# hzyu17/GaussianVI

Measured on AMD Instinct MI355X. Metric: sigma-point psi-evals/sec + NGD iters/sec, 1024-factor d=12 p=5 chain, higher is better.
Workload: dtype f64; 1 GPU; c3: T=1025 states, n=6; 1 step = 1 device-resident NGD iteration; restart every 30; factor_sets_columns=[K factors, d, GH degree p, N sigma points], factor_set_kinds=1024 x quadratic-prior d=12 p=5 (N=17217); 1025 x fixed-prior d=6 p=5 (N=1433), kernel_variant=6, chunks_per_factor=4, fused_pass=True, one_launch_factor_stage=False, mirror_pairs=False, fuse_trial=2

## Files before the change

gaussianvi_amd/csrc/chain_launch.hpp:

```cpp
#pragma once
#include <hip/hip_runtime.h>

#include <algorithm>
#include <atomic>
#include <vector>

#include "kernels_chain.hpp"
#include "kernels_chain_wave.hpp"

namespace gvi {

struct ChainPass { int level0, m, S, top, first, par, lp_off, blocks; };
struct ChainPlan { std::vector<ChainPass> passes; int threads = 0; };

inline int chain_padded(int n) {
  for (int N : {1, 2, 3, 4, 6, 8, 12, 16}) if (n <= N) return n >= 1 ? N : 0;
  return 0;
}
inline bool chain_supported(int n) { return chain_padded(n) != 0; }

inline int chain_levels(int T) {
  int L = 0;
  while ((1 << L) < T) ++L;
  return L;
// ... 20 lines not shown
  return p;
}

template <int N>
inline hipError_t chain_allow_lds() {
  static bool done[64] = {};
  int dev = 0;
  hipError_t e = hipGetDevice(&dev);
  if (e != hipSuccess) return e;
  if (dev >= 0 && dev < 64 && done[dev]) return hipSuccess;
  const int lim = 160 * 1024;
  if ((e = hipFuncSetAttribute((const void*)chain_forward_kernel<N, false>, hipFuncAttributeMaxDynamicSharedMemorySize, lim)) != hipSuccess) return e;
  if ((e = hipFuncSetAttribute((const void*)chain_forward_kernel<N, true>, hipFuncAttributeMaxDynamicSharedMemorySize, lim)) != hipSuccess) return e;
  if ((e = hipFuncSetAttribute((const void*)chain_backward_kernel<N>, hipFuncAttributeMaxDynamicSharedMemorySize, lim)) != hipSuccess) return e;
  if ((e = hipFuncSetAttribute((const void*)chain_top_back_kernel<N>, hipFuncAttributeMaxDynamicSharedMemorySize, lim)) != hipSuccess) return e;
  if (dev >= 0 && dev < 64) done[dev] = true;
  return hipSuccess;
}

struct ChainSync { unsigned* words = nullptr; unsigned seq = 0; unsigned fault = 0; };

template <int N>
inline hipError_t chain_launch_t(const ChainPlan& pl, ChainArgs a0, ChainArgs a1, bool on0, bool on1, hipStream_t st, const AsmList& AL,
                                 const ChainSync& sync) {
  hipError_t e = chain_allow_lds<N>();
  if (e != hipSuccess) return e;
  auto set = [](ChainArgs& a, const ChainPass& ps) {
    a.level0 = ps.level0; a.m = ps.m; a.S = ps.S; a.first = ps.first; a.par = ps.par; a.lp_off = ps.lp_off;
  };
  a0.sync = a1.sync = nullptr; a0.sync_seq = a1.sync_seq = 0; a0.sync_fault = a1.sync_fault = sync.fault;
  const bool back0 = on0 && a0.need_back;
  const int npass = (int)pl.passes.size();
  bool merged = false;
  if (sync.words && npass >= 2 && (back0 || on1)) {
    const ChainPass& pt = pl.passes[npass - 1];
    const ChainPass& pc = pl.passes[npass - 2];
    size_t lds = 0;
    if (on0) lds = std::max(lds, chain::fwd_lds_doubles<true, false, true, N>(pt.S));
    if (on1) lds = std::max(lds, chain::fwd_lds_doubles<false, true, true, N>(pt.S));
    if (back0) lds = std::max(lds, chain::bwd_lds_doubles<true, N>(pc.S));
    if (on1) lds = std::max(lds, chain::bwd_lds_doubles<false, N>(pc.S));
    merged = lds * 8 <= 160 * 1024;
  }
  for (const ChainPass& ps : pl.passes) {
    set(a0, ps); set(a1, ps);
    if (ps.top && merged) {
      const ChainPass& pc = pl.passes[npass - 2];
      size_t lds = 0;
      if (on0) lds = std::max(lds, chain::fwd_lds_doubles<true, false, true, N>(ps.S));
      if (on1) lds = std::max(lds, chain::fwd_lds_doubles<false, true, true, N>(ps.S));
      if (back0) lds = std::max(lds, chain::bwd_lds_doubles<true, N>(pc.S));
      if (on1) lds = std::max(lds, chain::bwd_lds_doubles<false, N>(pc.S));
      lds *= 8;
      a0.sync = sync.words; a1.sync = sync.words + 1; a0.sync_seq = a1.sync_seq = sync.seq;
      const int nb0 = on0 ? 1 : 0, nbt = nb0 + (on1 ? 1 : 0);
      const int nb0c = back0 ? pc.blocks : 0, nbc = nb0c + (on1 ? pc.blocks : 0);
      const ChainPassDev cp{pc.level0, pc.m, pc.S, pc.first, pc.par, pc.lp_off};
      hipLaunchKernelGGL((chain_top_back_kernel<N>), dim3(nbt + nbc), dim3(pl.threads), lds, st, a0, a1, nb0, AL, cp, nbt, nb0c);
      a0.sync = a1.sync = nullptr;
      continue;
    }
    size_t lds = 0;
    if (ps.top) {
      if (on0) lds = std::max(lds, chain::fwd_lds_doubles<true, false, true, N>(ps.S));
      if (on1) lds = std::max(lds, chain::fwd_lds_doubles<false, true, true, N>(ps.S));
    } else {
      if (on0) lds = std::max(lds, chain::fwd_lds_doubles<true, false, false, N>(ps.S));
      if (on1) lds = std::max(lds, chain::fwd_lds_doubles<false, true, false, N>(ps.S));
    }
    lds *= 8;
    if (lds > 160 * 1024) return hipErrorInvalidValue;
    const int nb0 = on0 ? ps.blocks : 0, nb = nb0 + (on1 ? ps.blocks : 0);
    if (ps.top) hipLaunchKernelGGL((chain_forward_kernel<N, true>), dim3(nb), dim3(pl.threads), lds, st, a0, a1, nb0, AL);
    else hipLaunchKernelGGL((chain_forward_kernel<N, false>), dim3(nb), dim3(pl.threads), lds, st, a0, a1, nb0, AL);
  }
  if (back0 || on1) {
    for (int i = npass - 2 - (merged ? 1 : 0); i >= 0; --i) {
      const ChainPass& ps = pl.passes[i];
      set(a0, ps); set(a1, ps);
      size_t lds = 0;
      if (back0) lds = std::max(lds, chain::bwd_lds_doubles<true, N>(ps.S));
      if (on1) lds = std::max(lds, chain::bwd_lds_doubles<false, N>(ps.S));
      lds *= 8;
      if (lds > 160 * 1024) return hipErrorInvalidValue;
      const int nb0 = back0 ? ps.blocks : 0, nb = nb0 + (on1 ? ps.blocks : 0);
      hipLaunchKernelGGL((chain_backward_kernel<N>), dim3(nb), dim3(pl.threads), lds, st, a0, a1, nb0);
    }
  }
  return hipGetLastError();
}

inline bool& chain_wave_enabled() { static bool on = true; return on; }
inline bool chain_wave_applies(int T, int n) { return chain_wave_enabled() && n >= 1 && n <= chain_wave::WN && T >= 1 && T <= chain_wave::WT_MAX; }

inline bool& chain_asm_dense_enabled() { static bool on = true; return on; }

inline std::atomic<long long>* chain_asm_launches() { static std::atomic<long long> c[2]; return c; }

inline hipError_t chain_launch(int n, const ChainPlan& pl, ChainArgs a0, ChainArgs a1, bool on0, bool on1, hipStream_t st,
                               const AsmList* AL = nullptr, const ChainSync& sync = ChainSync{}) {
  a0.n = a1.n = n;
  AsmList none{};
  const AsmList& L = AL ? *AL : none;
  if (!AL) a0.asm_on = a1.asm_on = 0;
  else if (chain_asm_dense_enabled() && chain_asm_dense(L, n) && (on0 ? a0.T : a1.T) > 1) {
    if (a0.asm_on) a0.asm_on = ASM_DENSE;
    if (a1.asm_on) a1.asm_on = ASM_DENSE;
    ++chain_asm_launches()[0];
  } else ++chain_asm_launches()[1];
  if (chain_wave_applies(on0 ? a0.T : a1.T, n)) {
    const int nb0 = on0 ? 1 : 0, nb = nb0 + (on1 ? 1 : 0);
    if (nb == 0) return hipSuccess;
    hipLaunchKernelGGL(chain_wave_kernel, dim3(nb), dim3(64), 0, st, a0, a1, nb0, L);
    return hipGetLastError();
  }
  switch (chain_padded(n)) {
// ... 14 lines not shown
```

gaussianvi_amd/csrc/gvi_hip.hip:

```cpp
#include "../../include/gvi_hip.h"

#include <hip/hip_runtime.h>
#include <hip/hip_ext.h>
#include <dlfcn.h>

#include <algorithm>
#include <chrono>
#include <cassert>
#include <cmath>
#include <cstdio>
#include <cstdlib>
#include <cstring>
#include <memory>
#include <map>
#include <set>
#include <string>
#include <thread>
#include <vector>

#include "host_linalg.hpp"
#include "kernels_bt.hpp"
#include "chain_launch.hpp"
#include "kernels_factor.hpp"
#include "kernels_orbit.hpp"
// ... 1009 lines not shown
  if (e != hipSuccess || ndev <= 0)
    return fail(nullptr, GVI_ERR_HIP, "no HIP device: this library has no CPU fallback");
  if (device < 0 || device >= ndev) return fail(nullptr, GVI_ERR_ARG, "device index out of range");
  if (hipSetDevice(device) != hipSuccess) return fail(nullptr, GVI_ERR_HIP, "hipSetDevice failed");
  std::unique_ptr<gvi_ctx> c(new gvi_ctx);
  c->device = device; c->dtype = dtype;
  if (hipStreamCreateWithFlags(&c->stream, hipStreamNonBlocking) != hipSuccess)
    return fail(nullptr, GVI_ERR_HIP, "hipStreamCreate failed");
  if (const char* w = getenv("GVI_NO_SCOST")) c->no_scost = atoi(w) != 0;
  if (const char* w = getenv("GVI_ORBIT")) c->orbit = atoi(w) != 0;
  if (const char* w = getenv("GVI_FUSED")) c->fused = atoi(w) != 0;
  if (const char* w = getenv("GVI_ASM_ON_LOAD")) c->asm_on_load = atoi(w) != 0;
  if (const char* w = getenv("GVI_PIPELINE")) c->pipeline = atoi(w) != 0;
  if (const char* w = getenv("GVI_CHAIN_WAVE")) chain_wave_enabled() = atoi(w) != 0;
  if (const char* w = getenv("GVI_ASM_DENSE")) chain_asm_dense_enabled() = atoi(w) != 0;
  if (const char* w = getenv("GVI_CHAIN_MERGE")) c->chain_merge = atoi(w) != 0;
  if (const char* w = getenv("GVI_SREG_PIPE")) c->sreg_pipe = atoi(w) != 0;
  if (const char* w = getenv("GVI_MIRROR")) c->mirror = atoi(w) != 0;
  if (const char* w = getenv("GVI_NO_PAIR")) c->pair_fuse = atoi(w) == 0;
  if (const char* w = getenv("GVI_NO_FUSE_GATHER")) c->fuse_gather = atoi(w) == 0;
  if (const char* w = getenv("GVI_SIDE_SOLVE")) c->side_solve = atoi(w) != 0;
  if (const char* w = getenv("GVI_FUSE_TRIAL")) c->fuse_trial = std::min(2, std::max(0, atoi(w)));
  if (const char* w = getenv("GVI_SPIN_MS")) c->spin_ms = std::max(0, atoi(w));
  if (const char* w = getenv("GVI_SAFE_PUBLISH")) c->safe_publish = atoi(w) != 0;
  if (hipEventCreateWithFlags(&c->fork, hipEventDisableTiming) != hipSuccess ||
      hipHostMalloc((void**)&c->host_slot, 128, hipHostMallocMapped | hipHostMallocCoherent) != hipSuccess ||
      hipHostGetDevicePointer((void**)&c->host_slot_dev, c->host_slot, 0) != hipSuccess)
    return fail(nullptr, GVI_ERR_HIP, "event / host-mapped slot allocation failed");
  for (int q = 0; q < 16; ++q) c->host_slot[q] = 0.0;
  *out = c.release();
// ... 2214 lines not shown
  else if (n == "sreg_pipe") ctx->sreg_pipe = value != 0;
  else if (n == "mirror") ctx->mirror = value != 0;
  else if (n == "pair_fuse") ctx->pair_fuse = value != 0;
  else if (n == "fuse_gather") ctx->fuse_gather = value != 0;
  else if (n == "side_solve") ctx->side_solve = value != 0;
  else if (n == "dual_chain") ctx->dual_chain = value != 0;
  else if (n == "warm_start") ctx->warm_start = value != 0;
  else if (n == "no_scost") ctx->no_scost = value != 0;
  else if (n == "target_waves") ctx->target_waves = std::max(1, value);
  else if (n == "orbit") ctx->orbit = value != 0;
  else if (n == "fused") ctx->fused = value != 0;
  else if (n == "assemble_on_load") ctx->asm_on_load = value != 0;
  else if (n == "pipeline") ctx->pipeline = value != 0;
  else if (n == "chain_wave") chain_wave_enabled() = value != 0;
  else if (n == "asm_dense") chain_asm_dense_enabled() = value != 0;
  else if (n == "sample_sweep") ctx->sample_sweep = value != 0;
  else if (n == "solve_lds") ctx->solve_lds = value != 0;
  else if (n == "chain_merge") { ctx->chain_merge = value != 0; ctx->chain_merge_fault = value == 2; }
  else if (n == "trust_table_degree") ctx->trust_table_degree = value != 0;
  else if (n == "safe_publish") {
    GVICK(sync(ctx));
    ctx->safe_publish = value != 0;
    for (int q = 0; q < 16; ++q) ctx->host_slot[q] = 0.0;
  }
  else if (n == "chol_sqrt") { ctx->chol_sqrt = value != 0; for (auto& s : ctx->sets) s->use_chol = ctx->chol_sqrt; }
  else if (n == "jacobi_tol_exp") {
    if (value > -20) return fail(ctx, GVI_ERR_ARG, "jacobi_tol_exp must be <= -20 (threshold 10^value on squared magnitudes)");
    ctx->jacobi_tol = std::pow(10.0, (double)value);
    for (auto& s : ctx->sets) s->jtol = ctx->jacobi_tol;
  }
// ... 330 lines not shown
```

gaussianvi_amd/csrc/kernels_chain.hpp:

```cpp
#pragma once
#include <hip/hip_runtime.h>
#include <stdint.h>

#include "device_common.hpp"
#include "kernels_bt.hpp"

namespace gvi {

constexpr int CHAIN_MATS = 10;
constexpr int CHAIN_VECS = 5;

__host__ __device__ inline size_t chain_lp_entries(int T) { return (size_t)2 * T + 1024; }
__host__ __device__ inline size_t chain_ws_doubles(int T, int n) {
  return (size_t)CHAIN_MATS * T * n * n + (size_t)CHAIN_VECS * T * n + chain_lp_entries(T);
}

struct ChainArgs {
  int T;
  int n;
  int level0;
  int m;
  int S;
  int first;
  int par;
  int need_back;
  int lp_off;
  const double* D;
  const double* U;
  const double* rhs;
  double rhs_scale;
  double* ws;
  int* wsi;
  double* SigD;
  double* SigU;
  double* x;
  double* hld;
  const double* mixV;
  double* mixOut;
  double mix_step;
  int asm_on;
  double* asmD;
// ... 187 lines not shown
}

__device__ __forceinline__ void st_out(double* p, const double v, const bool wt) {
  if (wt) __hip_atomic_store(p, v, __ATOMIC_RELAXED, __HIP_MEMORY_SCOPE_AGENT);
  else *p = v;
}

__device__ __forceinline__ double readlane64(double v, int src) {
  union { double d; int i[2]; } u;
  u.d = v;
  u.i[0] = __builtin_amdgcn_readlane(u.i[0], src);
  u.i[1] = __builtin_amdgcn_readlane(u.i[1], src);
  return u.d;
}

template <int N> __device__ __forceinline__ int ext_el(const int n, const int el) {
  if (n == N) return el;
  const int r = el / N, c = el % N;
  return (r < n && c < n) ? r * n + c : -1;
}

template <int N> __device__ __forceinline__ double* ws_mat(const ChainArgs& a, int idx) { return a.ws + (size_t)idx * a.T * (N * N); }
template <int N> __device__ __forceinline__ double* ws_vec(const ChainArgs& a, int idx) {
  return a.ws + (size_t)CHAIN_MATS * a.T * (N * N) + (size_t)idx * a.T * N;
}
template <int N> __device__ __forceinline__ double* ws_lp(const ChainArgs& a) { return ws_vec<N>(a, CHAIN_VECS); }
enum { W_E = 0, W_GA = 1, W_GB = 2, W_NU = 3, W_DEFF = 4, W_LS = 5 , W_RS = 7, W_SL = 8, W_SR = 9 };
enum { V_V = 0, V_YLS = 1 , V_YRS = 3, V_YEFF = 4 };

struct LogPiv {
// ... 9 lines not shown
  static constexpr int cY = cB + N;
  static constexpr int NC = cY + (HAS_Y ? 1 : 0);
  static_assert(NC <= 64, "tile does not fit one wave");
};

struct ElimIO {
  int oD, oR;
  int oUa, oUb;
  int oRa, oDb;
  int oNU;
  int oy, oyR, oyRa, oyb;
  int oZero;
  int oEl, oGAl, oGBl, ovl;
};

template <bool PIVOT, bool HAS_E, bool HAS_Y, bool TOP, int N>
__device__ __forceinline__ void eliminate(double* sm, const int lane, const ElimIO io, double* gE, double* gGA, double* gGB,
                                          double* gv, double* gNU, LogPiv& lp) {
  using C = Cols<HAS_E, HAS_Y, N>;
  const bool has_a = io.oUa >= 0, has_b = io.oUb >= 0;
  const bool isD = lane < N;
  const bool isE = HAS_E && lane >= C::cE && lane < C::cA;
  const bool isA = lane >= C::cA && lane < C::cB;
  const bool isB = lane >= C::cB && lane < C::cY;
  const bool isY = HAS_Y && lane == C::cY;
  const int cc = isD ? lane : (isE ? lane - C::cE : (isA ? lane - C::cA : (isB ? lane - C::cB : 0)));
  int p0 = io.oZero, s0 = 0, p1 = io.oZero;
  if (isD) { p0 = io.oD + cc * N; s0 = 1; p1 = io.oR + cc * N; }
  else if (isA) { if (has_a) { p0 = io.oUa + cc; s0 = N; } }
  else if (isB) { if (has_b) { p0 = io.oUb + cc * N; s0 = 1; } }
  else if (isY) { p0 = io.oy; s0 = 1; p1 = io.oyR; }
  CHAIN_STAMP(TOP && HAS_E);
  double col[N];
#pragma unroll
  for (int r = 0; r < N; ++r) col[r] = sm[p0 + r * s0] + sm[p1 + r];
  CHAIN_STAMP(TOP && HAS_E);
  if (HAS_E) {
#pragma unroll
    for (int r = 0; r < N; ++r) col[r] = isE ? (r == cc ? 1.0 : 0.0) : col[r];
  }
  constexpr int RB = chain_threads(N) == 1024 ? 128 : 256;
  constexpr bool PRE = N * N * 2 <= (RB == 128 ? 72 : 100);
  double uap[PRE ? N : 1][N];
  if (PRE && has_a) {
#pragma unroll
    for (int k = 0; k < (PRE ? N : 1); ++k) ld_row<N>(sm + io.oUa + k * N, uap[k]);
  }
  double pivs[N];
  int bad = 0;
#pragma unroll
  for (int p = 0; p < N; ++p) {
    if (PIVOT) {
      double best = fabs(col[p]);
      int rs = p;
#pragma unroll
      for (int r = p + 1; r < N; ++r) {
        const bool gt = fabs(col[r]) > best;
        best = gt ? fabs(col[r]) : best;
        rs = gt ? r : rs;
      }
      rs = fabs(col[p]) * 8.0 >= best ? p : rs;
      rs = __builtin_amdgcn_readlane(rs, p);
      if (rs != p) {
#pragma unroll
// ... 5 lines not shown
    double ap[N];
#pragma unroll
    for (int r = 0; r < N; ++r) ap[r] = readlane64(col[r], p);
    const double piv = ap[p];
    if (!(piv > 0.0)) bad = 1;
    pivs[p] = piv;
    double ip = __builtin_amdgcn_rcp(piv);
    ip = fma(fma(-piv, ip, 1.0), ip, ip);
    ip = fma(fma(-piv, ip, 1.0), ip, ip);
    const double f = col[p] * ip;
#pragma unroll
    for (int r = 0; r < N; ++r)
      if (r != p) col[r] = fma(-ap[r], f, col[r]);
    col[p] = f;
  }
  CHAIN_STAMP(TOP && HAS_E);
  {
    double mp = 1.0;
    int es = 0;
#pragma unroll
    for (int p = 0; p < N; ++p) {
      mp *= __builtin_amdgcn_frexp_mant(pivs[p]);
      es += __builtin_amdgcn_frexp_exp(pivs[p]);
    }
    const double t = lp.m * mp;
    lp.m = __builtin_amdgcn_frexp_mant(t);
    lp.e += es + __builtin_amdgcn_frexp_exp(t);
    lp.bad |= bad;
  }
  CHAIN_STAMP(TOP && HAS_E);
  if (TOP) {
    if (lane >= N && lane < C::NC) {
      const int o = isE ? io.oEl + cc : (isA ? io.oGAl + cc : (isB ? io.oGBl + cc : io.ovl));
      const int so = isY ? 1 : N;
#pragma unroll
      for (int r = 0; r < N; ++r) sm[o + r * so] = col[r];
    }
  } else {
    if (lane >= N && lane < C::NC) {
      double* g = isE ? gE + cc * N : (isA ? gGA + cc * N : (isB ? gGB + cc * N : gv));
      st_row<N>(g, col);
    }
  }
  CHAIN_STAMP(TOP && HAS_E);
  constexpr bool UBPRE = N * N * 2 <= (RB == 128 ? 32 : 100);
  double t[N], ub[UBPRE ? N : 1][N];
#pragma unroll
  for (int r = 0; r < N; ++r) t[r] = 0.0;
#pragma unroll
  for (int k = 0; k < N; ++k) {
    if (has_a) {
      double ua[N];
      if (PRE) {
#pragma unroll
// ... 34 lines not shown
#pragma unroll
        for (int k = 0; k < N; ++k) ubr[k] = ubl[UBLATE ? r : 0][k];
      } else ld_row<N>(sm + io.oUb + r * N, ubr);
      double acc = 0.0;
#pragma unroll
      for (int k = 0; k < N; ++k) acc = fma(-ubr[k], col[k], acc);
      s[r] = acc;
    }
    if (isB || isY) {
      double* o = sm + (isY ? io.oyb : io.oDb + cc * N);
#pragma unroll
      for (int r = 0; r < N; ++r) lds_add(o + r, s[r]);
    }
  }
  CHAIN_STAMP(TOP && HAS_E);
}

template <int N>
__device__ __forceinline__ void marginal_node(double* sm, const int lane, const bool has_b, const int oE, const int oGA, const int oGB,
                                              const int oSaa, const int oSbb, const int oX, const int oY, const int oSee,
                                              const int oSL, const int oSLt, const int oSR, const int oSRt, double* gSee, double* gSL,
                                              double* gSR, double* gUa, double* gUe, const int n,
                                              [[maybe_unused]] const bool stamp = false, const bool wt = false) {
  constexpr int nn = N * N, R = (nn + 63) / 64;
  double slv[R], srv[R];
  CHAIN_STAMP(stamp);
#pragma unroll
  for (int q = 0; q < R; ++q) {
    const int el = q * 64 + lane;
    const bool on = el < nn;
// ... 44 lines not shown
    if (has_b) {
      ld_row<N>(sm + oSR + r * N, u);
      ld_row<N>(sm + oGB + c * N, w);
#pragma unroll
      for (int k = 0; k < N; ++k) see = fma(-u[k], w[k], see);
    }
    if (on) {
      sm[oSee + el] = see;
      if (r < n && c < n) st_out(gSee + r * n + c, see, wt);
    }
  }
  CHAIN_STAMP(stamp);
}

template <bool HAS_E, bool HAS_Y, bool TOP, int N>
__host__ __device__ constexpr size_t fwd_lds_doubles(int S) {
  constexpr int nn = N * N;
  size_t w = (size_t)2 * (S + 1) * nn + (size_t)2 * S * nn;
  if (TOP) w += (size_t)3 * S * nn + (HAS_E ? (size_t)S * nn : 0);
  if (HAS_Y) w += (size_t)2 * (S + 1) * N + (TOP ? (size_t)(2 * S + 1) * N : 0);
  return w + N + (N & 1) + 128;
}
template <bool HAS_E, int N>
__host__ __device__ constexpr size_t bwd_lds_doubles(int S) {
  constexpr int nn = N * N;
  return (HAS_E ? (size_t)5 * (S + 1) * nn + (size_t)3 * S * nn
                : (size_t)(S + 1) * N + (size_t)S * N + (size_t)2 * S * nn)
         + 2;
}

__device__ __forceinline__ void chain_signal(unsigned* sync, const unsigned seq) {
  if (!sync) return;
  asm volatile("s_waitcnt vmcnt(0)" ::: "memory");
  __syncthreads();
  if (threadIdx.x == 0) __hip_atomic_store(sync, seq, __ATOMIC_RELAXED, __HIP_MEMORY_SCOPE_AGENT);
}
// ... 10 lines not shown
    *lds_word = ok;
  }
  __syncthreads();
  return *lds_word != 0;
}
__device__ __forceinline__ double chain_ld(const double* p, const bool fresh) {
  return fresh ? __hip_atomic_load(p, __ATOMIC_RELAXED, __HIP_MEMORY_SCOPE_AGENT) : *p;
}

__device__ __forceinline__ bool pred_fail_here(LazyPred& p) {
  __builtin_amdgcn_sched_barrier(0);
  asm volatile("" : "+v"(p.v));
  return pred_fail(p);
}

template <bool PIVOT, bool HAS_E, bool HAS_Y, bool TOP, int N>
__device__ __forceinline__ void forward_body(const ChainArgs& a, const AsmList& AL, const int bid, double* sm) {
  constexpr int nn = N * N;
  LazyPred lpred = pred_issue(a.pred, a.pred_val);
  const int T = a.T, S = a.S, st = 1 << a.level0;
  const int tid = threadIdx.x, wave = __builtin_amdgcn_readfirstlane(tid >> 6), lane = tid & 63, nwaves = blockDim.x >> 6, nthr = blockDim.x;
  const int x0 = bid * S * st;
  const int oDl = 0;
  const int oRl = oDl + (S + 1) * nn;
  const int oCt = oRl + (S + 1) * nn;
  const int oNU = oCt + S * nn;
  const int oEl = oNU + S * nn;
  const int oGAl = oEl + (TOP ? S * nn : 0);
  const int oGBl = oGAl + (TOP ? S * nn : 0);
  const int oSRt = oGBl + (TOP ? S * nn : 0);
  const int oyl = oSRt + ((TOP && HAS_E) ? S * nn : 0);
  const int oyR = oyl + (HAS_Y ? (S + 1) * N : 0);
  const int ovl = oyR + (HAS_Y ? (S + 1) * N : 0);
  const int oxl = ovl + ((HAS_Y && TOP) ? S * N : 0);
  const int oZero = oxl + ((HAS_Y && TOP) ? (S + 1) * N : 0);
  const int oRed = oZero + N + (N & 1);
  CHAIN_STAMP(TOP && HAS_E);
  const int cnt = min(S, (T - x0 + st - 1) >> a.level0);
  const int xn = x0 + S * st;
  const bool ext_right = !TOP && xn < T;
  const bool first = a.first != 0;
  const bool mix = first && (a.mixV != nullptr || (a.asm_on && !HAS_Y));
  [[maybe_unused]] double lpm = 1.0;
  [[maybe_unused]] int lpe = 0, lpb = 0;
  if constexpr (TOP) {
    if (a.hld) {
      for (int t = tid; t < a.lp_off; t += nthr) {
        const double mv = ws_lp<N>(a)[t];
        const int eb = a.wsi[t];
        const double pr = lpm * mv;
        lpm = __builtin_amdgcn_frexp_mant(pr);
// ... 169 lines not shown
#pragma unroll
      for (int o = 32; o > 0; o >>= 1) {
        const double t = lpm * __shfl_xor(lpm, o);
        lpe += __shfl_xor(lpe, o) + __builtin_amdgcn_frexp_exp(t);
        lpm = __builtin_amdgcn_frexp_mant(t);
        lpb |= __shfl_xor(lpb, o);
      }
      if (lane == 0) { sm[oRed + 64 + wave] = lpm; ((int*)(sm + oRed + 96))[wave] = lpe * 2 + lpb; }
    }
  }
  LogPiv lp;
  lp.m = 1.0; lp.e = 0; lp.bad = 0;
  for (int lam = 0; lam < a.m; ++lam) {
    const int h2 = 1 << lam;
    const int nel = (cnt + h2 - 1) >> (lam + 1);
    for (int u = wave; u < nel; u += nwaves) {
      const int j = (2 * u + 1) * h2, x = x0 + j * st;
      const int ja = j - h2, jb = j + h2;
      const bool has_b = (jb < cnt) || (jb == S && ext_right);
      ElimIO io;
      io.oD = oDl + j * nn; io.oR = oRl + j * nn;
      io.oUa = lam == 0 ? oCt + ja * nn : oNU + (j - h2 / 2) * nn;
      io.oUb = !has_b ? -1 : (lam == 0 ? oCt + j * nn : oNU + (j + h2 / 2) * nn);
      io.oRa = oRl + ja * nn; io.oDb = oDl + jb * nn;
      io.oNU = oNU + j * nn;
      io.oy = oyl + j * N; io.oyR = oyR + j * N; io.oyRa = oyR + ja * N; io.oyb = oyl + jb * N;
      io.oZero = oZero;
      io.oEl = oEl + j * nn; io.oGAl = oGAl + j * nn; io.oGBl = oGBl + j * nn; io.ovl = ovl + j * N;
      const size_t gx = (size_t)x * nn;
      double* gNU = (!TOP && lam == a.m - 1 && has_b) ? ws_mat<N>(a, W_NU) + gx : nullptr;
      eliminate<PIVOT, HAS_E, HAS_Y, TOP, N>(sm, lane, io, ws_mat<N>(a, W_E) + gx, ws_mat<N>(a, W_GA) + gx, ws_mat<N>(a, W_GB) + gx,
                                             ws_vec<N>(a, V_V) + (size_t)x * N, gNU, lp);
    }
    lds_barrier();
    CHAIN_STAMP(TOP && HAS_E);
  }
  if (!TOP) {
    for (int el = tid; el < nn; el += nthr) {
      ws_mat<N>(a, W_RS)[(size_t)x0 * nn + el] = sm[oRl + el];
      if (ext_right) ws_mat<N>(a, W_LS + a.par)[(size_t)xn * nn + el] = sm[oDl + S * nn + el];
    }
    if (HAS_Y && tid < N) {
      ws_vec<N>(a, V_YRS)[(size_t)x0 * N + tid] = sm[oyR + tid];
      if (ext_right) ws_vec<N>(a, V_YLS + a.par)[(size_t)xn * N + tid] = sm[oyl + S * N + tid];
    }
    if (lane == 0) {
      const int ent = a.lp_off + bid * nwaves + wave;
      ws_lp<N>(a)[ent] = lp.m;
      a.wsi[ent] = lp.e * 2 + lp.bad;
    }
    return;
  }
  if constexpr (TOP) {
    if (wave == 0) {
      ElimIO io;
      io.oD = oDl; io.oR = oRl; io.oUa = -1; io.oUb = -1; io.oRa = 0; io.oDb = 0; io.oNU = 0;
      io.oy = oyl; io.oyR = oyR; io.oyRa = 0; io.oyb = 0; io.oZero = oZero;
      io.oEl = oEl; io.oGAl = oGAl; io.oGBl = oGBl; io.ovl = ovl;
      eliminate<PIVOT, HAS_E, HAS_Y, true, N>(sm, lane, io, nullptr, nullptr, nullptr, nullptr, nullptr, lp);
    }
    int* redi = (int*)(sm + oRed + 32);
    if (a.hld && lane == 0) { sm[oRed + wave] = lp.m; redi[wave] = lp.e * 2 + lp.bad; }
    lds_barrier();
    if (a.hld && wave == nwaves - 1) {
      const int* redi2 = (const int*)(sm + oRed + 96);
      const int k2 = lane & 31;
      const bool on = k2 < nwaves;
      double mv = on ? (lane < 32 ? sm[oRed + k2] : sm[oRed + 64 + k2]) : 1.0;
      int eb = on ? (lane < 32 ? redi[k2] : redi2[k2]) : 0;
      int ev = eb >> 1, bflag = eb & 1;
#pragma unroll
      for (int o = 32; o > 0; o >>= 1) {
        const double t = mv * __shfl_xor(mv, o);
        ev += __shfl_xor(ev, o) + __builtin_amdgcn_frexp_exp(t);
// ... 214 lines not shown
      }
      lds_barrier();
    }
  }
}

}


template <int N, bool TOP>
__global__ __launch_bounds__(chain_threads(N)) void chain_forward_kernel(ChainArgs a0, ChainArgs a1, int nb0, AsmList AL) {
  extern __shared__ double sm[];
  constexpr int KA_LINES = (2 * sizeof(ChainArgs) + 8 + sizeof(AsmList) + 63) / 64;
  static_assert(KA_LINES == 13, "kernarg_warm: one specialisation per argument block size");
  kernarg_warm<KA_LINES>();
  if ((int)blockIdx.x < nb0) chain::forward_body<false, true, false, TOP, N>(a0, AL, (int)blockIdx.x, sm);
  else chain::forward_body<true, false, true, TOP, N>(a1, AL, (int)blockIdx.x - nb0, sm);
}

template <int N>
__global__ __launch_bounds__(chain_threads(N)) void chain_backward_kernel(ChainArgs a0, ChainArgs a1, int nb0) {
  extern __shared__ double sm[];
  constexpr int KA_LINES = (2 * sizeof(ChainArgs) + 4 + 63) / 64;
  static_assert(KA_LINES == 7, "kernarg_warm: one specialisation per argument block size");
  kernarg_warm<KA_LINES>();
  if ((int)blockIdx.x < nb0) chain::backward_body<true, false, N>(a0, (int)blockIdx.x, sm);
  else chain::backward_body<false, true, N>(a1, (int)blockIdx.x - nb0, sm);
}

template <int N>
__global__ __launch_bounds__(chain_threads(N)) void chain_top_back_kernel(ChainArgs a0, ChainArgs a1, int nb0, AsmList AL, ChainPassDev cp,
                                                                           int nbt, int nb0c) {
  extern __shared__ double sm[];
  constexpr int KA_LINES = (2 * sizeof(ChainArgs) + 8 + sizeof(AsmList) + sizeof(ChainPassDev) + 8 + 63) / 64;
  static_assert(KA_LINES == 14, "kernarg_warm: one specialisation per argument block size");
  kernarg_warm<KA_LINES>();
  const int b = (int)blockIdx.x;
  if (b < nbt) {
    if (b < nb0) chain::forward_body<false, true, false, true, N>(a0, AL, b, sm);
    else chain::forward_body<true, false, true, true, N>(a1, AL, b - nb0, sm);
    return;
  }
  const int bc = b - nbt;
  ChainArgs c = bc < nb0c ? a0 : a1;
  c.level0 = cp.level0; c.m = cp.m; c.S = cp.S; c.first = cp.first; c.par = cp.par; c.lp_off = cp.lp_off;
  if (bc < nb0c) chain::backward_body<true, false, N>(c, bc, sm);
  else chain::backward_body<false, true, N>(c, bc - nb0c, sm);
}

}
```

Before: 211.4 billion psi-evals/s.

## Add DPP row-broadcast Gauss-Jordan elimination with two eliminations per wave for n=6 chain

For padded block size 6, adds a new elimination path. Gauss-Jordan pivot broadcasts use DPP row_newbcast moves and fused v_fmac_f64_dpp instead of the previous per-pivot readlane-style broadcast. Columns are packed into a two-row 16-lane layout so each 64-lane wave handles two eliminations at once. The pivot log-determinant products are reduced through a small LDS scratch area. The old kernels are kept as readlane variants and selected per pass based on the ratio of eliminations to waves, and the feature can be toggled by env var or setting. This adds inline asm with s_nop hazard padding, extra LDS, and more template specialisations.

```diff
diff --git a/gaussianvi_amd/csrc/chain_launch.hpp b/gaussianvi_amd/csrc/chain_launch.hpp
--- a/gaussianvi_amd/csrc/chain_launch.hpp
+++ b/gaussianvi_amd/csrc/chain_launch.hpp
@@ -58,6 +58,11 @@
   if ((e = hipFuncSetAttribute((const void*)chain_forward_kernel<N, true>, hipFuncAttributeMaxDynamicSharedMemorySize, lim)) != hipSuccess) return e;
   if ((e = hipFuncSetAttribute((const void*)chain_backward_kernel<N>, hipFuncAttributeMaxDynamicSharedMemorySize, lim)) != hipSuccess) return e;
   if ((e = hipFuncSetAttribute((const void*)chain_top_back_kernel<N>, hipFuncAttributeMaxDynamicSharedMemorySize, lim)) != hipSuccess) return e;
+  if constexpr (N == 6) {
+    if ((e = hipFuncSetAttribute((const void*)chain_forward_readlane_kernel<false>, hipFuncAttributeMaxDynamicSharedMemorySize, lim)) != hipSuccess) return e;
+    if ((e = hipFuncSetAttribute((const void*)chain_forward_readlane_kernel<true>, hipFuncAttributeMaxDynamicSharedMemorySize, lim)) != hipSuccess) return e;
+    if ((e = hipFuncSetAttribute((const void*)chain_top_back_readlane_kernel, hipFuncAttributeMaxDynamicSharedMemorySize, lim)) != hipSuccess) return e;
+  }
   if (dev >= 0 && dev < 64) done[dev] = true;
   return hipSuccess;
 }
@@ -75,13 +80,15 @@
   a0.sync = a1.sync = nullptr; a0.sync_seq = a1.sync_seq = 0; a0.sync_fault = a1.sync_fault = sync.fault;
   const bool back0 = on0 && a0.need_back;
   const int npass = (int)pl.passes.size();
+  const bool pair_on = N == 6 && a0.pair != 0;
+  auto rowb = [&](const ChainPass& ps) { return pair_on && (ps.S >> 1) > pl.threads / 128; };
   bool merged = false;
   if (sync.words && npass >= 2 && (back0 || on1)) {
     const ChainPass& pt = pl.passes[npass - 1];
     const ChainPass& pc = pl.passes[npass - 2];
     size_t lds = 0;
-    if (on0) lds = std::max(lds, chain::fwd_lds_doubles<true, false, true, N>(pt.S));
-    if (on1) lds = std::max(lds, chain::fwd_lds_doubles<false, true, true, N>(pt.S));
+    if (on0) lds = std::max(lds, chain::fwd_lds_doubles<true, false, true, N>(pt.S, rowb(pt)));
+    if (on1) lds = std::max(lds, chain::fwd_lds_doubles<false, true, true, N>(pt.S, rowb(pt)));
     if (back0) lds = std::max(lds, chain::bwd_lds_doubles<true, N>(pc.S));
     if (on1) lds = std::max(lds, chain::bwd_lds_doubles<false, N>(pc.S));
     merged = lds * 8 <= 160 * 1024;
@@ -91,8 +98,8 @@
     if (ps.top && merged) {
       const ChainPass& pc = pl.passes[npass - 2];
       size_t lds = 0;
-      if (on0) lds = std::max(lds, chain::fwd_lds_doubles<true, false, true, N>(ps.S));
-      if (on1) lds = std::max(lds, chain::fwd_lds_doubles<false, true, true, N>(ps.S));
+      if (on0) lds = std::max(lds, chain::fwd_lds_doubles<true, false, true, N>(ps.S, rowb(ps)));
+      if (on1) lds = std::max(lds, chain::fwd_lds_doubles<false, true, true, N>(ps.S, rowb(ps)));
       if (back0) lds = std::max(lds, chain::bwd_lds_doubles<true, N>(pc.S));
       if (on1) lds = std::max(lds, chain::bwd_lds_doubles<false, N>(pc.S));
       lds *= 8;
@@ -100,21 +107,34 @@
       const int nb0 = on0 ? 1 : 0, nbt = nb0 + (on1 ? 1 : 0);
       const int nb0c = back0 ? pc.blocks : 0, nbc = nb0c + (on1 ? pc.blocks : 0);
       const ChainPassDev cp{pc.level0, pc.m, pc.S, pc.first, pc.par, pc.lp_off};
-      hipLaunchKernelGGL((chain_top_back_kernel<N>), dim3(nbt + nbc), dim3(pl.threads), lds, st, a0, a1, nb0, AL, cp, nbt, nb0c);
+      bool launched = false;
+      if constexpr (N == 6) {
+        if (!rowb(ps)) { hipLaunchKernelGGL(chain_top_back_readlane_kernel, dim3(nbt + nbc), dim3(pl.threads), lds, st, a0, a1, nb0, AL, cp, nbt, nb0c); launched = true; }
+      }
+      if (!launched) hipLaunchKernelGGL((chain_top_back_kernel<N>), dim3(nbt + nbc), dim3(pl.threads), lds, st, a0, a1, nb0, AL, cp, nbt, nb0c);
       a0.sync = a1.sync = nullptr;
       continue;
     }
     size_t lds = 0;
     if (ps.top) {
-      if (on0) lds = std::max(lds, chain::fwd_lds_doubles<true, false, true, N>(ps.S));
-      if (on1) lds = std::max(lds, chain::fwd_lds_doubles<false, true, true, N>(ps.S));
+      if (on0) lds = std::max(lds, chain::fwd_lds_doubles<true, false, true, N>(ps.S, rowb(ps)));
+      if (on1) lds = std::max(lds, chain::fwd_lds_doubles<false, true, true, N>(ps.S, rowb(ps)));
     } else {
-      if (on0) lds = std::max(lds, chain::fwd_lds_doubles<true, false, false, N>(ps.S));
-      if (on1) lds = std::max(lds, chain::fwd_lds_doubles<false, true, false, N>(ps.S));
+      if (on0) lds = std::max(lds, chain::fwd_lds_doubles<true, false, false, N>(ps.S, rowb(ps)));
+      if (on1) lds = std::max(lds, chain::fwd_lds_doubles<false, true, false, N>(ps.S, rowb(ps)));
     }
     lds *= 8;
     if (lds > 160 * 1024) return hipErrorInvalidValue;
     const int nb0 = on0 ? ps.blocks : 0, nb = nb0 + (on1 ? ps.blocks : 0);
+    bool launched = false;
+    if constexpr (N == 6) {
+      if (!rowb(ps)) {
+        if (ps.top) hipLaunchKernelGGL(chain_forward_readlane_kernel<true>, dim3(nb), dim3(pl.threads), lds, st, a0, a1, nb0, AL);
+        else hipLaunchKernelGGL(chain_forward_readlane_kernel<false>, dim3(nb), dim3(pl.threads), lds, st, a0, a1, nb0, AL);
+        launched = true;
+      }
+    }
+    if (launched) continue;
     if (ps.top) hipLaunchKernelGGL((chain_forward_kernel<N, true>), dim3(nb), dim3(pl.threads), lds, st, a0, a1, nb0, AL);
     else hipLaunchKernelGGL((chain_forward_kernel<N, false>), dim3(nb), dim3(pl.threads), lds, st, a0, a1, nb0, AL);
   }
@@ -139,11 +159,14 @@
 
 inline bool& chain_asm_dense_enabled() { static bool on = true; return on; }
 
+inline bool& chain_pair_enabled() { static bool on = true; return on; }
+
 inline std::atomic<long long>* chain_asm_launches() { static std::atomic<long long> c[2]; return c; }
 
 inline hipError_t chain_launch(int n, const ChainPlan& pl, ChainArgs a0, ChainArgs a1, bool on0, bool on1, hipStream_t st,
                                const AsmList* AL = nullptr, const ChainSync& sync = ChainSync{}) {
   a0.n = a1.n = n;
+  a0.pair = a1.pair = chain_pair_enabled() ? 1 : 0;
   AsmList none{};
   const AsmList& L = AL ? *AL : none;
   if (!AL) a0.asm_on = a1.asm_on = 0;
diff --git a/gaussianvi_amd/csrc/gvi_hip.hip b/gaussianvi_amd/csrc/gvi_hip.hip
--- a/gaussianvi_amd/csrc/gvi_hip.hip
+++ b/gaussianvi_amd/csrc/gvi_hip.hip
@@ -1047,6 +1047,7 @@
   if (const char* w = getenv("GVI_PIPELINE")) c->pipeline = atoi(w) != 0;
   if (const char* w = getenv("GVI_CHAIN_WAVE")) chain_wave_enabled() = atoi(w) != 0;
   if (const char* w = getenv("GVI_ASM_DENSE")) chain_asm_dense_enabled() = atoi(w) != 0;
+  if (const char* w = getenv("GVI_CHAIN_PAIR")) chain_pair_enabled() = atoi(w) != 0;
   if (const char* w = getenv("GVI_CHAIN_MERGE")) c->chain_merge = atoi(w) != 0;
   if (const char* w = getenv("GVI_SREG_PIPE")) c->sreg_pipe = atoi(w) != 0;
   if (const char* w = getenv("GVI_MIRROR")) c->mirror = atoi(w) != 0;
@@ -3291,6 +3292,7 @@
   else if (n == "pipeline") ctx->pipeline = value != 0;
   else if (n == "chain_wave") chain_wave_enabled() = value != 0;
   else if (n == "asm_dense") chain_asm_dense_enabled() = value != 0;
+  else if (n == "chain_pair") chain_pair_enabled() = value != 0;
   else if (n == "sample_sweep") ctx->sample_sweep = value != 0;
   else if (n == "solve_lds") ctx->solve_lds = value != 0;
   else if (n == "chain_merge") { ctx->chain_merge = value != 0; ctx->chain_merge_fault = value == 2; }
diff --git a/gaussianvi_amd/csrc/kernels_chain.hpp b/gaussianvi_amd/csrc/kernels_chain.hpp
--- a/gaussianvi_amd/csrc/kernels_chain.hpp
+++ b/gaussianvi_amd/csrc/kernels_chain.hpp
@@ -25,6 +25,7 @@
   int par;
   int need_back;
   int lp_off;
+  int pair;
   const double* D;
   const double* U;
   const double* rhs;
@@ -242,6 +243,21 @@
   return u.d;
 }
 
+template <int P, int WS>
+__device__ __forceinline__ double rowb_mov(const double v) {
+  double o;
+  if constexpr (WS > 1) asm volatile("s_nop 4\n\tv_mov_b64_dpp %0, %1 row_newbcast:%2 row_mask:0xf bank_mask:0xf" : "=v"(o) : "v"(v), "n"(P));
+  else asm volatile("s_nop 1\n\tv_mov_b64_dpp %0, %1 row_newbcast:%2 row_mask:0xf bank_mask:0xf" : "=v"(o) : "v"(v), "n"(P));
+  return o;
+}
+template <int P>
+__device__ __forceinline__ void rowb_fmac(double& c, const double b) {
+  asm volatile("v_fmac_f64_dpp %0, %0, %1 row_newbcast:%2 row_mask:0xf bank_mask:0xf" : "+v"(c) : "v"(b), "n"(P));
+}
+__device__ __forceinline__ void rowb_pin(double& v) { asm volatile("" : "+v"(v)); }
+template <int P>
+__device__ __forceinline__ int rowb_int(const int v) { return __builtin_amdgcn_update_dpp(0, v, 0x150 + P, 0xf, 0xf, false); }
+
 template <int N> __device__ __forceinline__ int ext_el(const int n, const int el) {
   if (n == N) return el;
   const int r = el / N, c = el % N;
@@ -281,17 +297,80 @@
   int oEl, oGAl, oGBl, ovl;
 };
 
-template <bool PIVOT, bool HAS_E, bool HAS_Y, bool TOP, int N>
+template <bool PIVOT, int N, int P>
+__device__ __forceinline__ void gj_rowb(double (&col)[N], double& mp, int& es, int& bad) {
+  if constexpr (P < N) {
+    if (PIVOT) {
+      double best = fabs(col[P]);
+      int rs = P;
+#pragma unroll
+      for (int r = P + 1; r < N; ++r) {
+        const bool gt = fabs(col[r]) > best;
+        best = gt ? fabs(col[r]) : best;
+        rs = gt ? r : rs;
+      }
+      rs = fabs(col[P]) * 8.0 >= best ? P : rs;
+      rs = rowb_int<P>(rs);
+      if (__builtin_amdgcn_ballot_w64(rs != P) != 0) {
+#pragma unroll
+        for (int r = P + 1; r < N; ++r) {
+          const bool sw = r == rs;
+          const double t = col[P];
+          col[P] = sw ? col[r] : t;
+          col[r] = sw ? t : col[r];
+        }
+      }
+    }
+    if (PIVOT || P == 0) {
+#pragma unroll
+      for (int r = 0; r < N; ++r) rowb_pin(col[r]);
+    }
+    const double piv = rowb_mov<P, PIVOT ? 4 : 1>(col[P]);
+    if (!(piv > 0.0)) bad = 1;
+    mp *= __builtin_amdgcn_frexp_mant(piv);
+    es += __builtin_amdgcn_frexp_exp(piv);
+    double ip = __builtin_amdgcn_rcp(piv);
+    ip = fma(fma(-piv, ip, 1.0), ip, ip);
+    ip = fma(fma(-piv, ip, 1.0), ip, ip);
+    double f = col[P] * ip;
+    rowb_pin(f);
+    const double nf = -f;
+#pragma unroll
+    for (int r = 0; r < N; ++r)
+      if (r != P) rowb_fmac<P>(col[r], nf);
+    col[P] = f;
+    gj_rowb<PIVOT, N, P + 1>(col, mp, es, bad);
+  }
+}
+
+template <bool PIVOT, bool HAS_E, bool HAS_Y, bool TOP, int N, bool ROWB = false>
 __device__ __forceinline__ void eliminate(double* sm, const int lane, const ElimIO io, double* gE, double* gGA, double* gGB,
                                           double* gv, double* gNU, LogPiv& lp) {
   using C = Cols<HAS_E, HAS_Y, N>;
   const bool has_a = io.oUa >= 0, has_b = io.oUb >= 0;
-  const bool isD = lane < N;
-  const bool isE = HAS_E && lane >= C::cE && lane < C::cA;
-  const bool isA = lane >= C::cA && lane < C::cB;
-  const bool isB = lane >= C::cB && lane < C::cY;
-  const bool isY = HAS_Y && lane == C::cY;
-  const int cc = isD ? lane : (isE ? lane - C::cE : (isA ? lane - C::cA : (isB ? lane - C::cB : 0)));
+  bool isD, isE, isA, isB, isY;
+  int cc;
+  if constexpr (ROWB) {
+    constexpr int G0 = 16 - 2 * N;
+    static_assert(!ROWB || (G0 > 0 && G0 <= N && 2 * N - G0 + (HAS_E ? N : 1) <= 16), "two-row layout");
+    constexpr int l1 = 16 + N, l2 = l1 + N - G0;
+    const bool split0 = lane >= 16 - G0 && lane < 16, split1 = lane >= l1 && lane < l2;
+    isD = lane < N || (lane >= 16 && lane < l1);
+    isE = HAS_E && lane >= N && lane < 2 * N;
+    isA = HAS_E ? (split0 || split1) : (lane >= N && lane < 2 * N);
+    isB = HAS_E ? (lane >= l2 && lane < l2 + N) : (split0 || split1);
+    isY = HAS_Y && lane == l2;
+    const int cs = split0 ? lane - (16 - G0) : lane - l1 + G0;
+    cc = isD ? (lane < N ? lane : lane - 16) : (isE ? lane - N : (isA ? (HAS_E ? cs : lane - N) : (isB ? (HAS_E ? lane - l2 : cs) : 0)));
+  } else {
+    isD = lane < N;
+    isE = HAS_E && lane >= C::cE && lane < C::cA;
+    isA = lane >= C::cA && lane < C::cB;
+    isB = lane >= C::cB && lane < C::cY;
+    isY = HAS_Y && lane == C::cY;
+    cc = isD ? lane : (isE ? lane - C::cE : (isA ? lane - C::cA : (isB ? lane - C::cB : 0)));
+  }
+  const bool isF = ROWB ? (isE || isA || isB || isY) : (lane >= N && lane < C::NC);
   int p0 = io.oZero, s0 = 0, p1 = io.oZero;
   if (isD) { p0 = io.oD + cc * N; s0 = 1; p1 = io.oR + cc * N; }
   else if (isA) { if (has_a) { p0 = io.oUa + cc; s0 = N; } }
@@ -313,8 +392,11 @@
 #pragma unroll
     for (int k = 0; k < (PRE ? N : 1); ++k) ld_row<N>(sm + io.oUa + k * N, uap[k]);
   }
+  double mp = 1.0;
+  int es = 0, bad = 0;
+  if constexpr (ROWB) gj_rowb<PIVOT, N, 0>(col, mp, es, bad);
+  else {
   double pivs[N];
-  int bad = 0;
 #pragma unroll
   for (int p = 0; p < N; ++p) {
     if (PIVOT) {
@@ -350,15 +432,14 @@
       if (r != p) col[r] = fma(-ap[r], f, col[r]);
     col[p] = f;
   }
+#pragma unroll
+  for (int p = 0; p < N; ++p) {
+    mp *= __builtin_amdgcn_frexp_mant(pivs[p]);
+    es += __builtin_amdgcn_frexp_exp(pivs[p]);
+  }
+  }
   CHAIN_STAMP(TOP && HAS_E);
   {
-    double mp = 1.0;
-    int es = 0;
-#pragma unroll
-    for (int p = 0; p < N; ++p) {
-      mp *= __builtin_amdgcn_frexp_mant(pivs[p]);
-      es += __builtin_amdgcn_frexp_exp(pivs[p]);
-    }
     const double t = lp.m * mp;
     lp.m = __builtin_amdgcn_frexp_mant(t);
     lp.e += es + __builtin_amdgcn_frexp_exp(t);
@@ -366,14 +447,14 @@
   }
   CHAIN_STAMP(TOP && HAS_E);
   if (TOP) {
-    if (lane >= N && lane < C::NC) {
+    if (isF) {
       const int o = isE ? io.oEl + cc : (isA ? io.oGAl + cc : (isB ? io.oGBl + cc : io.ovl));
       const int so = isY ? 1 : N;
 #pragma unroll
       for (int r = 0; r < N; ++r) sm[o + r * so] = col[r];
     }
   } else {
-    if (lane >= N && lane < C::NC) {
+    if (isF) {
       double* g = isE ? gE + cc * N : (isA ? gGA + cc * N : (isB ? gGB + cc * N : gv));
       st_row<N>(g, col);
     }
@@ -438,6 +519,96 @@
     }
   }
   CHAIN_STAMP(TOP && HAS_E);
+}
+
+struct ElimBases {
+  int oDl, oRl, oCt, oNU, oEl, oGAl, oGBl, ovl, oyl, oyR, oZero;
+};
+template <bool PIVOT, bool HAS_E, bool HAS_Y, bool TOP, int N>
+__device__ __forceinline__ void eliminate2(double* sm, const int lane, const int jv, const int slot, const bool lam0, const int h2,
+                                           const bool has_b, const ElimBases B, double* wE, double* wGA, double* wGB, double* wv,
+                                           const int st, const int olp) {
+  constexpr int nn = N * N;
+  constexpr int G0 = 16 - 2 * N, l1 = 16 + N, l2 = l1 + N - G0;
+  static_assert(G0 > 0 && G0 <= N && 2 * N - G0 + (HAS_E ? N : 1) <= 16, "two-row layout");
+  const int l = lane & 31;
+  const bool on = jv >= 0;
+  const int j = on ? jv : h2;
+  const bool split0 = l >= 16 - G0 && l < 16, split1 = l >= l1 && l < l2;
+  const bool isD = on && (l < N || (l >= 16 && l < l1));
+  const bool isE = on && HAS_E && l >= N && l < 2 * N;
+  const bool isA = on && (HAS_E ? (split0 || split1) : (l >= N && l < 2 * N));
+  const bool isB = on && (HAS_E ? (l >= l2 && l < l2 + N) : (split0 || split1));
+  const bool isY = on && HAS_Y && l == l2;
+  const int cs = split0 ? l - (16 - G0) : l - l1 + G0;
+  const int cc = isD ? (l < N ? l : l - 16) : (isE ? l - N : (isA ? (HAS_E ? cs : l - N) : (isB ? (HAS_E ? l - l2 : cs) : 0)));
+  const bool isF = isE || isA || isB || isY;
+  const int ja = j - h2, jb = j + h2;
+  const int oUa = lam0 ? B.oCt + ja * nn : B.oNU + (j - h2 / 2) * nn;
+  int p0 = B.oZero, s0 = 0, p1 = B.oZero;
+  if (isD) { p0 = B.oDl + j * nn + cc * N; s0 = 1; p1 = B.oRl + j * nn + cc * N; }
+  else if (isA) { p0 = oUa + cc; s0 = N; }
+  else if (isB) { if (has_b) { p0 = (lam0 ? B.oCt + j * nn : B.oNU + (j + h2 / 2) * nn) + cc * N; s0 = 1; } }
+  else if (isY) { p0 = B.oyl + j * N; s0 = 1; p1 = B.oyR + j * N; }
+  double col[N];
+#pragma unroll
+  for (int r = 0; r < N; ++r) col[r] = sm[p0 + r * s0] + sm[p1 + r];
+  if (HAS_E) {
+#pragma unroll
+    for (int r = 0; r < N; ++r) col[r] = isE ? (r == cc ? 1.0 : 0.0) : col[r];
+  }
+  double mp = 1.0;
+  int es = 0, bad = 0;
+  gj_rowb<PIVOT, N, 0>(col, mp, es, bad);
+  __builtin_amdgcn_sched_barrier(0);
+  double uap[N][N];
+#pragma unroll
+  for (int k = 0; k < N; ++k) ld_row<N>(sm + oUa + k * N, uap[k]);
+  if (on && l == 0) { sm[olp + slot] = mp; ((int*)(sm + olp + 32))[slot] = es * 2 + bad; }
+  if (isF) {
+    if (TOP) {
+      const int o = (isE ? B.oEl + cc : (isA ? B.oGAl + cc : (isB ? B.oGBl + cc : B.ovl))) + j * (isY ? N : nn);
+      const int so = isY ? 1 : N;
+#pragma unroll
+      for (int r = 0; r < N; ++r) sm[o + r * so] = col[r];
+    } else {
+      const size_t xo = (size_t)j * st;
+      double* g = isY ? wv + xo * N : (isE ? wE : (isA ? wGA : wGB)) + xo * nn + cc * N;
+      st_row<N>(g, col);
+    }
+  }
+  double t[N];
+#pragma unroll
+  for (int r = 0; r < N; ++r) t[r] = 0.0;
+#pragma unroll
+  for (int k = 0; k < N; ++k) {
+#pragma unroll
+    for (int r = 0; r < N; ++r) t[r] = fma(-uap[k][r], col[k], t[r]);
+  }
+  const int oUb = lam0 ? B.oCt + j * nn : B.oNU + (j + h2 / 2) * nn;
+  double ubl[N][N];
+#pragma unroll
+  for (int r = 0; r < N; ++r) ld_row<N>(sm + oUb + r * N, ubl[r]);
+  __builtin_amdgcn_sched_barrier(0);
+  if (isA || isY) {
+    double* o = sm + (isY ? B.oyR + ja * N : B.oRl + ja * nn + cc * N);
+#pragma unroll
+    for (int r = 0; r < N; ++r) lds_add(o + r, t[r]);
+  }
+  if (has_b && isB) st_row<N>(sm + B.oNU + j * nn + cc * N, t);
+  double sv[N];
+#pragma unroll
+  for (int r = 0; r < N; ++r) {
+    double acc = 0.0;
+#pragma unroll
+    for (int k = 0; k < N; ++k) acc = fma(-ubl[r][k], col[k], acc);
+    sv[r] = acc;
+  }
+  if (has_b && (isB || isY)) {
+    double* o = sm + (isY ? B.oyl + jb * N : B.oDl + jb * nn + cc * N);
+#pragma unroll
+    for (int r = 0; r < N; ++r) lds_add(o + r, sv[r]);
+  }
 }
 
 template <int N>
@@ -512,12 +683,12 @@
 }
 
 template <bool HAS_E, bool HAS_Y, bool TOP, int N>
-__host__ __device__ constexpr size_t fwd_lds_doubles(int S) {
+__host__ __device__ constexpr size_t fwd_lds_doubles(int S, bool rowb = false) {
   constexpr int nn = N * N;
   size_t w = (size_t)2 * (S + 1) * nn + (size_t)2 * S * nn;
   if (TOP) w += (size_t)3 * S * nn + (HAS_E ? (size_t)S * nn : 0);
   if (HAS_Y) w += (size_t)2 * (S + 1) * N + (TOP ? (size_t)(2 * S + 1) * N : 0);
-  return w + N + (N & 1) + 128;
+  return w + N + (N & 1) + 128 + (rowb ? 96 : 0);
 }
 template <bool HAS_E, int N>
 __host__ __device__ constexpr size_t bwd_lds_doubles(int S) {
@@ -558,7 +729,7 @@
   return pred_fail(p);
 }
 
-template <bool PIVOT, bool HAS_E, bool HAS_Y, bool TOP, int N>
+template <bool PIVOT, bool HAS_E, bool HAS_Y, bool TOP, int N, bool ROWB = false>
 __device__ __forceinline__ void forward_body(const ChainArgs& a, const AsmList& AL, const int bid, double* sm) {
   constexpr int nn = N * N;
   LazyPred lpred = pred_issue(a.pred, a.pred_val);
@@ -579,6 +750,7 @@
   const int oxl = ovl + ((HAS_Y && TOP) ? S * N : 0);
   const int oZero = oxl + ((HAS_Y && TOP) ? (S + 1) * N : 0);
   const int oRed = oZero + N + (N & 1);
+  [[maybe_unused]] const int oLp2 = oRed + 128;
   CHAIN_STAMP(TOP && HAS_E);
   const int cnt = min(S, (T - x0 + st - 1) >> a.level0);
   const int xn = x0 + S * st;
@@ -778,6 +950,33 @@
   for (int lam = 0; lam < a.m; ++lam) {
     const int h2 = 1 << lam;
     const int nel = (cnt + h2 - 1) >> (lam + 1);
+    if constexpr (ROWB) {
+      if (nel > nwaves / 2 && nel <= 32) {
+        const int npair = (nel + 1) >> 1, half = lane >> 5;
+        const int olp = oLp2 + (lam & 1) * 48;
+        const ElimBases EB{oDl, oRl, oCt, oNU, oEl, oGAl, oGBl, ovl, oyl, oyR, oZero};
+        for (int q = wave; q < npair; q += nwaves) {
+          const int u = q + half * npair;
+          const int jv = u < nel ? (2 * u + 1) * h2 : -1;
+          const bool has_b = jv >= 0 && ((jv + h2 < cnt) || (jv + h2 == S && ext_right));
+          const size_t go = (size_t)x0 * nn;
+          eliminate2<PIVOT, HAS_E, HAS_Y, TOP, N>(sm, lane, jv, u, lam == 0, h2, has_b, EB, TOP ? nullptr : ws_mat<N>(a, W_E) + go,
+                                                  TOP ? nullptr : ws_mat<N>(a, W_GA) + go, TOP ? nullptr : ws_mat<N>(a, W_GB) + go,
+                                                  TOP ? nullptr : ws_vec<N>(a, V_V) + (size_t)x0 * N, st, olp);
+        }
+        lds_barrier();
+        for (int u = wave; u < nel; u += nwaves) {
+          const double mp = sm[olp + u];
+          const int eb = ((const int*)(sm + olp + 32))[u];
+          const double t = lp.m * mp;
+          lp.m = __builtin_amdgcn_frexp_mant(t);
+          lp.e += (eb >> 1) + __builtin_amdgcn_frexp_exp(t);
+          lp.bad |= eb & 1;
+        }
+        CHAIN_STAMP(TOP && HAS_E);
+        continue;
+      }
+    }
     for (int u = wave; u < nel; u += nwaves) {
       const int j = (2 * u + 1) * h2, x = x0 + j * st;
       const int ja = j - h2, jb = j + h2;
@@ -793,8 +992,8 @@
       io.oEl = oEl + j * nn; io.oGAl = oGAl + j * nn; io.oGBl = oGBl + j * nn; io.ovl = ovl + j * N;
       const size_t gx = (size_t)x * nn;
       double* gNU = (!TOP && lam == a.m - 1 && has_b) ? ws_mat<N>(a, W_NU) + gx : nullptr;
-      eliminate<PIVOT, HAS_E, HAS_Y, TOP, N>(sm, lane, io, ws_mat<N>(a, W_E) + gx, ws_mat<N>(a, W_GA) + gx, ws_mat<N>(a, W_GB) + gx,
-                                             ws_vec<N>(a, V_V) + (size_t)x * N, gNU, lp);
+      eliminate<PIVOT, HAS_E, HAS_Y, TOP, N, ROWB>(sm, lane, io, ws_mat<N>(a, W_E) + gx, ws_mat<N>(a, W_GA) + gx, ws_mat<N>(a, W_GB) + gx,
+                                                   ws_vec<N>(a, V_V) + (size_t)x * N, gNU, lp);
     }
     lds_barrier();
     CHAIN_STAMP(TOP && HAS_E);
@@ -821,7 +1020,7 @@
       io.oD = oDl; io.oR = oRl; io.oUa = -1; io.oUb = -1; io.oRa = 0; io.oDb = 0; io.oNU = 0;
       io.oy = oyl; io.oyR = oyR; io.oyRa = 0; io.oyb = 0; io.oZero = oZero;
       io.oEl = oEl; io.oGAl = oGAl; io.oGBl = oGBl; io.ovl = ovl;
-      eliminate<PIVOT, HAS_E, HAS_Y, true, N>(sm, lane, io, nullptr, nullptr, nullptr, nullptr, nullptr, lp);
+      eliminate<PIVOT, HAS_E, HAS_Y, true, N, ROWB>(sm, lane, io, nullptr, nullptr, nullptr, nullptr, nullptr, lp);
     }
     int* redi = (int*)(sm + oRed + 32);
     if (a.hld && lane == 0) { sm[oRed + wave] = lp.m; redi[wave] = lp.e * 2 + lp.bad; }
@@ -1066,8 +1265,8 @@
   constexpr int KA_LINES = (2 * sizeof(ChainArgs) + 8 + sizeof(AsmList) + 63) / 64;
   static_assert(KA_LINES == 13, "kernarg_warm: one specialisation per argument block size");
   kernarg_warm<KA_LINES>();
-  if ((int)blockIdx.x < nb0) chain::forward_body<false, true, false, TOP, N>(a0, AL, (int)blockIdx.x, sm);
-  else chain::forward_body<true, false, true, TOP, N>(a1, AL, (int)blockIdx.x - nb0, sm);
+  if ((int)blockIdx.x < nb0) chain::forward_body<false, true, false, TOP, N, N == 6>(a0, AL, (int)blockIdx.x, sm);
+  else chain::forward_body<true, false, true, TOP, N, N == 6>(a1, AL, (int)blockIdx.x - nb0, sm);
 }
 
 template <int N>
@@ -1089,8 +1288,8 @@
   kernarg_warm<KA_LINES>();
   const int b = (int)blockIdx.x;
   if (b < nbt) {
-    if (b < nb0) chain::forward_body<false, true, false, true, N>(a0, AL, b, sm);
-    else chain::forward_body<true, false, true, true, N>(a1, AL, b - nb0, sm);
+    if (b < nb0) chain::forward_body<false, true, false, true, N, N == 6>(a0, AL, b, sm);
+    else chain::forward_body<true, false, true, true, N, N == 6>(a1, AL, b - nb0, sm);
     return;
   }
   const int bc = b - nbt;
@@ -1100,4 +1299,29 @@
   else chain::backward_body<false, true, N>(c, bc - nb0c, sm);
 }
 
-}
+template <bool TOP>
+__global__ __launch_bounds__(chain_threads(6)) void chain_forward_readlane_kernel(ChainArgs a0, ChainArgs a1, int nb0, AsmList AL) {
+  extern __shared__ double sm[];
+  kernarg_warm<13>();
+  if ((int)blockIdx.x < nb0) chain::forward_body<false, true, false, TOP, 6, false>(a0, AL, (int)blockIdx.x, sm);
+  else chain::forward_body<true, false, true, TOP, 6, false>(a1, AL, (int)blockIdx.x - nb0, sm);
+}
+
+__global__ __launch_bounds__(chain_threads(6)) void chain_top_back_readlane_kernel(ChainArgs a0, ChainArgs a1, int nb0, AsmList AL,
+                                                                                  ChainPassDev cp, int nbt, int nb0c) {
+  extern __shared__ double sm[];
+  kernarg_warm<14>();
+  const int b = (int)blockIdx.x;
+  if (b < nbt) {
+    if (b < nb0) chain::forward_body<false, true, false, true, 6, false>(a0, AL, b, sm);
+    else chain::forward_body<true, false, true, true, 6, false>(a1, AL, b - nb0, sm);
+    return;
+  }
+  const int bc = b - nbt;
+  ChainArgs c = bc < nb0c ? a0 : a1;
+  c.level0 = cp.level0; c.m = cp.m; c.S = cp.S; c.first = cp.first; c.par = cp.par; c.lp_off = cp.lp_off;
+  if (bc < nb0c) chain::backward_body<true, false, 6>(c, bc, sm);
+  else chain::backward_body<false, true, 6>(c, bc - nb0c, sm);
+}
+
+}
```

After: 214.5 billion psi-evals/s (median of 6 runs). +1.5%, better.
